# awentzonline/tartangan

Hardware: AMD Instinct MI355X
Metric: images/sec (G+D step) (higher is better)
Workload: dtype f32; 1 GPU; 128:3 SA-GAN cnn G+D step (R1 penalty, Adam x2, EMA), 128x128 RGB, batch 64/GPU, global batch 64; trainer=cnn, gan_config=128:3, global_batch=64, parallelism=dp1, hip_graphs=True

## Files before the change

tartangan_amd/csrc/conv.hip:

```cpp
#include <cstdlib>
#include <type_traits>
#include <utility>

#include "common.h"

namespace {

typedef float f32x16 __attribute__((ext_vector_type(16)));
typedef float f32x4 __attribute__((ext_vector_type(4)));

constexpr int CT_THREADS = 256;

template <int TH_, int TW_, int NI_>
struct Geo {
  static constexpr int TH = TH_, TW = TW_, NI = NI_, NPIX = TH_ * TW_ * NI_;
  static_assert(NPIX == 512 || NPIX == 256 || NPIX == 64, "a pixel tile is 512 / 256 pixels (waves split pixels) or 64 (waves split K)");
  static constexpr int PPW = (NPIX == 64) ? 64 : NPIX / 4;
  static_assert(TW_ % 4 == 0, "rows are staged as float4");
};
using G4 = Geo<4, 4, 16>;
using G8 = Geo<8, 8, 4>;
using G16 = Geo<16, 16, 1>;
using GX = Geo<8, 32, 1>;
using G4k = Geo<4, 4, 4>;
// ... 1033 lines not shown
  for (int n = 0; n < NT; ++n) {
    const int col = n * 16 + j;
    const int ci = col / KK, tap = col % KK;
    colbase[n] = (col < C::NCOL) ? (ci * P::CIS + (tap / KS) * P::PWS + (tap % KS)) : 0;
  }
  const int lane_b = pix_off<G, KS>(wave * 64) + h;
  const int lane_a = j * WG_GYS + wave * 64 + h;

  f32x4 acc[MTW][NT];
#pragma unroll
  for (int m = 0; m < MTW; ++m)
#pragma unroll
    for (int n = 0; n < NT; ++n) acc[m][n] = f32x4{0.f, 0.f, 0.f, 0.f};

  PatchStager<G, KS, CKW> ps;
  GyStager<G, CT> gs;
  const bool do_bias = (bias_part != nullptr) && (blockIdx.z == 0);
  float bsum[GyStager<G, CT>::NV];
#pragma unroll
  for (int i = 0; i < GyStager<G, CT>::NV; ++i) bsum[i] = 0.f;
  if (split < ntiles) {
    const TileCoord tc = decode_tile<G>(split, s.H, s.W);
    ps.load(x, s, s.Cin, ci0, tc, vec_x);
    gs.load(gy, s, co0, tc, vec_gy);
  }
  for (int t = split; t < ntiles; t += S) {
    __syncthreads();
    ps.store(pl);
    gs.store(gl);
    if (do_bias) gs.add_channel_sums(bsum);
    __syncthreads();
    if (t + S < ntiles) {
      const TileCoord tn = decode_tile<G>(t + S, s.H, s.W);
      ps.load(x, s, s.Cin, ci0, tn, vec_x);
      gs.load(gy, s, co0, tn, vec_gy);
    }
#pragma unroll
    for (int g = 0; g < 16; ++g) {
      constexpr int PPI = G::TH * G::TW;
      const int pg = 4 * g;
      const int goff = ((pg / PPI) * P::PH + (pg % PPI) / G::TW) * P::PWS + (pg % G::TW);
      float a[MTW], b[NT];
#pragma unroll
      for (int m = 0; m < MTW; ++m) a[m] = gl[lane_a + m * 16 * WG_GYS + 4 * g];
#pragma unroll
      for (int n = 0; n < NT; ++n) b[n] = pl[colbase[n] + lane_b + goff];
#pragma unroll
      for (int m = 0; m < MTW; ++m)
#pragma unroll
        for (int n = 0; n < NT; ++n) acc[m][n] = __builtin_amdgcn_mfma_f32_16x16x4f32(a[m], b[n], acc[m][n], 0, 0, 0);
    }
  }

  if (do_bias && lane == 0) {
#pragma unroll
    for (int i = 0; i < GyStager<G, CT>::NV; ++i) {
      const int co = co0 + 4 * i + wave;
      if (4 * i + wave < CT && co < s.Cout) bias_part[(int64_t)split * s.Cout + co] = bsum[i];
    }
  }
  __syncthreads();
  float* red = lds;
#pragma unroll
  for (int m = 0; m < MTW; ++m)
#pragma unroll
    for (int n = 0; n < NT; ++n)
#pragma unroll
      for (int r = 0; r < 4; ++r) red[(((wave * MTW + m) * NT + n) * 4 + r) * 64 + lane] = acc[m][n][r];
  __syncthreads();
  constexpr int PER_WAVE = MTW * NT * 4 * 64;
  for (int e = threadIdx.x; e < PER_WAVE; e += CT_THREADS) {
    const float v = (red[e] + red[PER_WAVE + e]) + (red[2 * PER_WAVE + e] + red[3 * PER_WAVE + e]);
    const int l = e & 63, q = e >> 6;
    const int r = q & 3, n = (q >> 2) % NT, m = (q >> 2) / NT;
    const int col = n * 16 + (l & 15);
    const int co = co0 + m * 16 + (l >> 4) * 4 + r;
    const int ci = ci0 + col / KK, tap = col % KK;
    if (col < C::NCOL && co < s.Cout && ci < s.Cin)
      part[(((int64_t)split * s.Cout + co) * s.Cin + ci) * KK + tap] = v;
  }
}

constexpr int WGD_GYQ = 65;
template <class G, int MTW, int CKW, bool DB>
__global__ void __launch_bounds__(CT_THREADS)
conv_wgrad_dma_kernel(const float* __restrict__ x, const float* __restrict__ gy, float* __restrict__ part,
                      float* __restrict__ bias_part , Shape s, int ntiles, int S) {
  static_assert(G::NPIX == 256 && WG_GYS == 4 * WGD_GYQ, "256-pixel tiles");
  using P = DPatch<G>;
  constexpr int KK = 9, CT = 16 * MTW, NCOL = CKW * KK, NT = (NCOL + 15) / 16;
  constexpr int PCH = CKW * P::CPC, GCH = CT * WGD_GYQ;
  constexpr int PCHP = dma_pad(PCH), GCHP = dma_pad(GCH);
  constexpr int NVP = (PCHP + CT_THREADS - 1) / CT_THREADS, NVG = (GCHP + CT_THREADS - 1) / CT_THREADS;
  constexpr int PBUF = PCHP * 4, BUF = PBUF + GCHP * 4;
  constexpr int RED = 4 * MTW * NT * 4 * 64 + 4 * CT;
  constexpr int LDSF = ((DB ? 2 : 1) * BUF > RED) ? (DB ? 2 : 1) * BUF : RED;
  __shared__ __attribute__((aligned(16))) float lds[LDSF];

  const int lane = threadIdx.x & 63, wave = wave_index();
  if (s.prio) __builtin_amdgcn_s_setprio(3);
  const int j = lane & 15, h = lane >> 4;
  const int co0 = blockIdx.y * CT, ci0 = blockIdx.z * CKW;
  const int split = blockIdx.x;
  const uint32_t HW = (uint32_t)(s.H * s.W);

  int colbase[NT];
#pragma unroll
  for (int n = 0; n < NT; ++n) {
    const int col = n * 16 + j;
    const int ci = col / KK, tap = col % KK;
    colbase[n] = (col < NCOL) ? (ci * P::CIS + (tap / 3) * P::PWS + (tap % 3)) : 0;
  }
  const int lane_b = P::pix(wave * 64) + h;
  const int lane_a = j * WG_GYS + wave * 64 + h;

  f32x4 acc[MTW][NT];
#pragma unroll
  for (int m = 0; m < MTW; ++m)
#pragma unroll
    for (int n = 0; n < NT; ++n) acc[m][n] = f32x4{0.f, 0.f, 0.f, 0.f};
  const bool do_bias = (bias_part != nullptr) && (blockIdx.z == 0);
  float bsum[MTW];
#pragma unroll
  for (int m = 0; m < MTW; ++m) bsum[m] = 0.f;

  const int cvalid = min(CKW, s.Cin - ci0);
  auto issue = [&](int t, float* buf) {
    const TileCoord tc = decode_tile<G>(t, s.H, s.W);
    const char* xb = reinterpret_cast<const char*>(x) + ((int64_t)tc.b0 * s.Cin + ci0) * HW * 4;
    const int64_t xbytes = ((int64_t)(s.B - tc.b0) * s.Cin - ci0) * HW * 4;
    const char* gb = reinterpret_cast<const char*>(gy) + ((int64_t)tc.b0 * s.Cout + co0) * HW * 4;
    const int64_t gbytes = ((int64_t)(s.B - tc.b0) * s.Cout - co0) * HW * 4;
    const __amdgpu_buffer_rsrc_t rx = __builtin_amdgcn_make_buffer_rsrc(const_cast<char*>(xb), 0, (int)xbytes, 0x00020000);
    const __amdgpu_buffer_rsrc_t rg = __builtin_amdgcn_make_buffer_rsrc(const_cast<char*>(gb), 0, (int)gbytes, 0x00020000);
#pragma unroll
    for (int i = 0; i < NVP; ++i) {
      const int e = i * CT_THREADS + threadIdx.x;
      const int ci = e / P::CPC, rem = e % P::CPC;
      const int row = rem / P::QR, q = rem % P::QR;
      const int img = row / P::PH, r = row % P::PH;
      const int hh = tc.h0 + r - 1, ww = tc.w0 - 4 + 4 * q;
      const bool ok = (rem < P::RAW / 4) && (ci < cvalid) && (tc.b0 + img < s.B) && (hh >= 0) && (hh < s.H) && (ww >= 0) && (ww < s.W);
      const uint32_t off = ok ? (__umul24(__umul24(img, s.Cin) + ci, HW) + __umul24(hh, s.W) + ww) << 2 : DMA_OOB;
      if ((i + 1) * CT_THREADS <= PCHP || i * CT_THREADS + wave * 64 < PCHP) dma16(rx, buf + (i * CT_THREADS + wave * 64) * 4, off);
    }
#pragma unroll
    for (int i = 0; i < NVG; ++i) {
      const int e = i * CT_THREADS + threadIdx.x;
      const int co = e / WGD_GYQ, q = e % WGD_GYQ;
      const int p = 4 * q;
      const int img = p / (G::TH * G::TW), rem = p % (G::TH * G::TW);
      const int hh = tc.h0 + rem / G::TW, ww = tc.w0 + rem % G::TW;
      const bool ok = (e < GCH) && (q < 64) && (co0 + co < s.Cout) && (tc.b0 + img < s.B) && (hh < s.H) && (ww < s.W);
      const uint32_t off = ok ? (__umul24(__umul24(img, s.Cout) + co, HW) + __umul24(hh, s.W) + ww) << 2 : DMA_OOB;
      if ((i + 1) * CT_THREADS <= GCHP || i * CT_THREADS + wave * 64 < GCHP) dma16(rg, buf + PBUF + (i * CT_THREADS + wave * 64) * 4, off);
    }
  };
  auto compute = [&](const float* buf) {
    const float* pl = buf;
    const float* gl = buf + PBUF;
    if (s.prio) __builtin_amdgcn_s_setprio(0);
#pragma unroll
    for (int g = 0; g < 16; ++g) {
      constexpr int PPI = G::TH * G::TW;
      const int pg = 4 * g;
      const int goff = ((pg / PPI) * P::PH + (pg % PPI) / G::TW) * P::PWS + (pg % G::TW);
      float a[MTW], b[NT];
#pragma unroll
      for (int m = 0; m < MTW; ++m) a[m] = gl[lane_a + m * 16 * WG_GYS + 4 * g];
#pragma unroll
      for (int n = 0; n < NT; ++n) b[n] = pl[colbase[n] + lane_b + goff];
#pragma unroll
      for (int m = 0; m < MTW; ++m) bsum[m] += a[m];
#pragma unroll
      for (int m = 0; m < MTW; ++m)
#pragma unroll
        for (int n = 0; n < NT; ++n) acc[m][n] = __builtin_amdgcn_mfma_f32_16x16x4f32(a[m], b[n], acc[m][n], 0, 0, 0);
    }
    if (s.prio) __builtin_amdgcn_s_setprio(3);
  };

  if constexpr (DB) {
    if (split < ntiles) issue(split, lds);
    int buf = 0;
    for (int t = split; t < ntiles; t += S) {
      asm volatile("s_waitcnt vmcnt(0)" ::: "memory");
      __syncthreads();
      if (t + S < ntiles) issue(t + S, lds + (buf ^ 1) * BUF);
      compute(lds + buf * BUF);
      buf ^= 1;
    }
  } else {
    for (int t = split; t < ntiles; t += S) {
      __syncthreads();
      issue(t, lds);
      asm volatile("s_waitcnt vmcnt(0)" ::: "memory");
      __syncthreads();
      compute(lds);
    }
  }

  __syncthreads();
  float* red = lds;
#pragma unroll
  for (int m = 0; m < MTW; ++m)
#pragma unroll
    for (int n = 0; n < NT; ++n)
#pragma unroll
      for (int r = 0; r < 4; ++r) red[(((wave * MTW + m) * NT + n) * 4 + r) * 64 + lane] = acc[m][n][r];
  constexpr int PER_WAVE = MTW * NT * 4 * 64;
  float* bred = lds + 4 * PER_WAVE;
  if (do_bias) {
#pragma unroll
    for (int m = 0; m < MTW; ++m) {
      float v = bsum[m];
      v += __shfl_xor(v, 16, 64);
      v += __shfl_xor(v, 32, 64);
      if (h == 0) bred[wave * CT + m * 16 + j] = v;
    }
  }
  __syncthreads();
  for (int e = threadIdx.x; e < PER_WAVE; e += CT_THREADS) {
    const float v = (red[e] + red[PER_WAVE + e]) + (red[2 * PER_WAVE + e] + red[3 * PER_WAVE + e]);
    const int l = e & 63, q = e >> 6;
    const int r = q & 3, n = (q >> 2) % NT, m = (q >> 2) / NT;
    const int col = n * 16 + (l & 15);
    const int co = co0 + m * 16 + (l >> 4) * 4 + r;
    const int ci = ci0 + col / KK, tap = col % KK;
    if (col < NCOL && co < s.Cout && ci < s.Cin)
      part[(((int64_t)split * s.Cout + co) * s.Cin + ci) * KK + tap] = v;
  }
  if (do_bias && threadIdx.x < CT && co0 + (int)threadIdx.x < s.Cout) {
    const int c = threadIdx.x;
    bias_part[(int64_t)split * s.Cout + co0 + c] = (bred[c] + bred[CT + c]) + (bred[2 * CT + c] + bred[3 * CT + c]);
  }
}

template <int MT, int NT>
__global__ void __launch_bounds__(256)
conv1x1_wgrad_stream_kernel(const float* __restrict__ x, ChanSegs gys, float* __restrict__ part,
                            float* __restrict__ bias_part , int Cin, int Cout, int HW, int64_t groups, int S) {
  __shared__ float red[4 * MT * NT * 4 * 64 + 4 * 16 * MT];
  const int lane = threadIdx.x & 63, wave = threadIdx.x >> 6, j = lane & 15, h = lane >> 4;
  const int co0 = blockIdx.y * 16 * MT, ci0 = blockIdx.z * 16 * NT, split = blockIdx.x;
  const int64_t g_begin = groups * split / S, g_end = groups * (split + 1) / S;
  const int64_t n = g_end - g_begin;
  const int64_t w_begin = g_begin + n * wave / 4, w_end = g_begin + n * (wave + 1) / 4;
  const int gpp = HW >> 4;
  int64_t arow[MT], brow[NT], aimg[MT];
  const float* abase[MT];
#pragma unroll
  for (int m = 0; m < MT; ++m) {
    const int co = min(co0 + 16 * m + j, Cout - 1), k = gys.find(co);
    abase[m] = gys.p[k];
// ... 894 lines not shown
                     float* __restrict__ bias_part , int bias_mode) {
  using P = Patch2x<G>;
  constexpr int CKW = S2_CKW, NT = S2_NT, CT = 16;
  constexpr int PATCH = CKW * P::CIS, GYT = CT * WG_GYS;
  constexpr int RED = 4 * NT * 4 * 64;
  constexpr int LDS_FLOATS = (PATCH + GYT) > RED ? (PATCH + GYT) : RED;
  __shared__ __attribute__((aligned(16))) float lds[LDS_FLOATS];
  float* pl = lds;
  float* gl = lds + PATCH;
  const int lane = threadIdx.x & 63, wave = threadIdx.x >> 6;
  const int j = lane & 15, h = lane >> 4;
  const int co0 = blockIdx.y * CT, ci0 = blockIdx.z * CKW;
  const int split = blockIdx.x;
  int colbase[NT];
#pragma unroll
  for (int n = 0; n < NT; ++n) colbase[n] = n * P::CIS + (j >> 2) * P::PWS + (j & 3);
  const int lane_b = P::pix(wave * 64) + 2 * h;
  const int lane_a = j * WG_GYS + wave * 64 + h;
  f32x4 acc[NT];
  float bsum_a = 0.f, bsum_b[NT];
#pragma unroll
  for (int n = 0; n < NT; ++n) { acc[n] = f32x4{0.f, 0.f, 0.f, 0.f}; bsum_b[n] = 0.f; }
  const bool do_bias = bias_part != nullptr && (bias_mode == 0 ? blockIdx.z == 0 : blockIdx.y == 0);
  auto products = [&](const float* pl, const float* gl, auto with_sums) {
#pragma unroll
    for (int g = 0; g < 16; ++g) {
      const int pg = 4 * g;
      const int goff = 2 * (pg / G::TW) * P::PWS + 2 * (pg % G::TW);
      const float a = gl[lane_a + 4 * g];
      float b[NT];
#pragma unroll
      for (int n = 0; n < NT; ++n) b[n] = pl[colbase[n] + lane_b + goff];
      if constexpr (decltype(with_sums)::value) {
        bsum_a += a;
#pragma unroll
        for (int n = 0; n < NT; ++n) bsum_b[n] += b[n];
      }
#pragma unroll
      for (int n = 0; n < NT; ++n) acc[n] = __builtin_amdgcn_mfma_f32_16x16x4f32(a, b[n], acc[n], 0, 0, 0);
    }
  };
  PatchStager2x<G, CKW> ps;
  GyStager<G, CT> gs;
  const int H2 = 2 * s.H, W2 = 2 * s.W;
  if (split < ntiles) {
    const TileCoord tc = decode_tile<G>(split, s.H, s.W);
    ps.load(hi, s.B, s.Cin, H2, W2, ci0, tc, vec_hi);
    gs.load(lo, s, co0, tc, vec_lo);
  }
  for (int t = split; t < ntiles; t += S) {
    __syncthreads();
    ps.store(pl);
    gs.store(gl);
    __syncthreads();
    if (t + S < ntiles) {
      const TileCoord tn = decode_tile<G>(t + S, s.H, s.W);
      ps.load(hi, s.B, s.Cin, H2, W2, ci0, tn, vec_hi);
      gs.load(lo, s, co0, tn, vec_lo);
    }
    if (do_bias) products(pl, gl, std::true_type{});
    else products(pl, gl, std::false_type{});
  }
  __syncthreads();
  float* red = lds;
#pragma unroll
  for (int n = 0; n < NT; ++n)
#pragma unroll
    for (int r = 0; r < 4; ++r) red[((wave * NT + n) * 4 + r) * 64 + lane] = acc[n][r];
  __syncthreads();
  constexpr int PER_WAVE = NT * 4 * 64;
  for (int e = threadIdx.x; e < PER_WAVE; e += CT_THREADS) {
    const float v = (red[e] + red[PER_WAVE + e]) + (red[2 * PER_WAVE + e] + red[3 * PER_WAVE + e]);
    const int l = e & 63, q = e >> 6;
    const int r = q & 3, n = q >> 2;
    const int co = co0 + (l >> 4) * 4 + r, ci = ci0 + n, tap = l & 15;
    if (co < s.Cout && ci < s.Cin) part[(((int64_t)split * s.Cout + co) * s.Cin + ci) * 16 + tap] = v;
  }
  if (do_bias) {
    __syncthreads();
    s2_bias_finish<NT>(red, bsum_a, bsum_b, bias_mode, bias_part, split, s.Cout, s.Cin, co0, ci0, lane, wave);
  }
}

template <class G>
__global__ void __launch_bounds__(CT_THREADS)
conv_wgrad_s2_dma_kernel(const float* __restrict__ hi, const float* __restrict__ lo, float* __restrict__ part, Shape s , int ntiles, int S, float* __restrict__ bias_part ,
                         int bias_mode) {
  static_assert(G::NPIX == 256, "256-pixel tiles");
  using P = DPatch2x<G>;
  constexpr int CKW = S2_CKW, NT = S2_NT, CT = 16;
  constexpr int PCH = CKW * P::CPC, GCH = CT * WGD_GYQ;
  constexpr int PCHP = dma_pad(PCH), GCHP = dma_pad(GCH);
  constexpr int NVP = (PCHP + CT_THREADS - 1) / CT_THREADS, NVG = (GCHP + CT_THREADS - 1) / CT_THREADS;
  constexpr int PBUF = PCHP * 4, BUF = PBUF + GCHP * 4;
  constexpr int RED = 4 * NT * 4 * 64;
  __shared__ __attribute__((aligned(16))) float lds[BUF > RED ? BUF : RED];
  const int lane = threadIdx.x & 63, wave = wave_index();
  if (s.prio) __builtin_amdgcn_s_setprio(3);
  const int j = lane & 15, h = lane >> 4;
  const int co0 = blockIdx.y * CT, ci0 = blockIdx.z * CKW;
  const int split = blockIdx.x;
  const int H2 = 2 * s.H, W2 = 2 * s.W;
  const uint32_t HW = (uint32_t)(s.H * s.W), HW2 = (uint32_t)(H2 * W2);
  int colbase[NT];
#pragma unroll
  for (int n = 0; n < NT; ++n) colbase[n] = n * P::CIS + (j >> 2) * P::PWS + (j & 3);
  const int lane_b = P::pix(wave * 64) + 2 * h;
  const int lane_a = j * WG_GYS + wave * 64 + h;
  f32x4 acc[NT];
  float bsum_a = 0.f, bsum_b[NT];
#pragma unroll
  for (int n = 0; n < NT; ++n) { acc[n] = f32x4{0.f, 0.f, 0.f, 0.f}; bsum_b[n] = 0.f; }
  const bool do_bias = bias_part != nullptr && (bias_mode == 0 ? blockIdx.z == 0 : blockIdx.y == 0);
  auto products = [&](const float* pl, const float* gl, auto with_sums) {
#pragma unroll
    for (int g = 0; g < 16; ++g) {
      const int pg = 4 * g;
      const int goff = 2 * (pg / G::TW) * P::PWS + 2 * (pg % G::TW);
      const float a = gl[lane_a + 4 * g];
      float b[NT];
#pragma unroll
      for (int n = 0; n < NT; ++n) b[n] = pl[colbase[n] + lane_b + goff];
      if constexpr (decltype(with_sums)::value) {
        bsum_a += a;
#pragma unroll
        for (int n = 0; n < NT; ++n) bsum_b[n] += b[n];
      }
#pragma unroll
      for (int n = 0; n < NT; ++n) acc[n] = __builtin_amdgcn_mfma_f32_16x16x4f32(a, b[n], acc[n], 0, 0, 0);
    }
  };
  const int cvalid = min(CKW, s.Cin - ci0);
  for (int t = split; t < ntiles; t += S) {
    const TileCoord tc = decode_tile<G>(t, s.H, s.W);
    const char* xb = reinterpret_cast<const char*>(hi) + ((int64_t)tc.b0 * s.Cin + ci0) * HW2 * 4;
    const int64_t xbytes = ((int64_t)(s.B - tc.b0) * s.Cin - ci0) * HW2 * 4;
    const char* gb = reinterpret_cast<const char*>(lo) + ((int64_t)tc.b0 * s.Cout + co0) * HW * 4;
    const int64_t gbytes = ((int64_t)(s.B - tc.b0) * s.Cout - co0) * HW * 4;
    const __amdgpu_buffer_rsrc_t rx = __builtin_amdgcn_make_buffer_rsrc(const_cast<char*>(xb), 0, (int)xbytes, 0x00020000);
    const __amdgpu_buffer_rsrc_t rg = __builtin_amdgcn_make_buffer_rsrc(const_cast<char*>(gb), 0, (int)gbytes, 0x00020000);
    __syncthreads();
#pragma unroll
    for (int i = 0; i < NVP; ++i) {
      const int e = i * CT_THREADS + threadIdx.x;
      const int ci = e / P::CPC, rem = e % P::CPC;
      const int row = rem / P::QR, q = rem % P::QR;
      const int img = row / P::PH, r = row % P::PH;
      const int hh = 2 * tc.h0 - 1 + r, ww = 2 * tc.w0 - 4 + 4 * q;
      const bool ok = (rem < P::RAW / 4) && (ci < cvalid) && (tc.b0 + img < s.B) && (hh >= 0) && (hh < H2) && (ww >= 0) && (ww < W2);
      const uint32_t off = ok ? (__umul24(__umul24(img, s.Cin) + ci, HW2) + __umul24(hh, W2) + ww) << 2 : DMA_OOB;
      if ((i + 1) * CT_THREADS <= PCHP || i * CT_THREADS + wave * 64 < PCHP) dma16(rx, lds + (i * CT_THREADS + wave * 64) * 4, off);
    }
#pragma unroll
    for (int i = 0; i < NVG; ++i) {
      const int e = i * CT_THREADS + threadIdx.x;
      const int co = e / WGD_GYQ, q = e % WGD_GYQ;
      const int p = 4 * q;
      const int img = p / (G::TH * G::TW), rem = p % (G::TH * G::TW);
      const int hh = tc.h0 + rem / G::TW, ww = tc.w0 + rem % G::TW;
      const bool ok = (e < GCH) && (q < 64) && (co0 + co < s.Cout) && (tc.b0 + img < s.B) && (hh < s.H) && (ww < s.W);
      const uint32_t off = ok ? (__umul24(__umul24(img, s.Cout) + co, HW) + __umul24(hh, s.W) + ww) << 2 : DMA_OOB;
      if ((i + 1) * CT_THREADS <= GCHP || i * CT_THREADS + wave * 64 < GCHP) dma16(rg, lds + PBUF + (i * CT_THREADS + wave * 64) * 4, off);
    }
    asm volatile("s_waitcnt vmcnt(0)" ::: "memory");
    __syncthreads();
    const float* pl = lds;
    const float* gl = lds + PBUF;
    if (s.prio) __builtin_amdgcn_s_setprio(0);
    if (do_bias) products(pl, gl, std::true_type{});
    else products(pl, gl, std::false_type{});
    if (s.prio) __builtin_amdgcn_s_setprio(3);
  }
  __syncthreads();
  float* red = lds;
#pragma unroll
  for (int n = 0; n < NT; ++n)
#pragma unroll
    for (int r = 0; r < 4; ++r) red[((wave * NT + n) * 4 + r) * 64 + lane] = acc[n][r];
  __syncthreads();
  constexpr int PER_WAVE = NT * 4 * 64;
  for (int e = threadIdx.x; e < PER_WAVE; e += CT_THREADS) {
    const float v = (red[e] + red[PER_WAVE + e]) + (red[2 * PER_WAVE + e] + red[3 * PER_WAVE + e]);
    const int l = e & 63, q = e >> 6;
    const int r = q & 3, n = q >> 2;
    const int co = co0 + (l >> 4) * 4 + r, ci = ci0 + n, tap = l & 15;
    if (co < s.Cout && ci < s.Cin) part[(((int64_t)split * s.Cout + co) * s.Cin + ci) * 16 + tap] = v;
  }
  if (do_bias) {
    __syncthreads();
    s2_bias_finish<NT>(red, bsum_a, bsum_b, bias_mode, bias_part, split, s.Cout, s.Cin, co0, ci0, lane, wave);
  }
}

__device__ __forceinline__ void s2wgrad_reduce_fold(const float* __restrict__ part, float* __restrict__ gw, int S, int Clo, int Chi,
                                                    int Cout, int Cin, int mode, int accumulate,
                                                    const float* __restrict__ bias_part , float* __restrict__ gbias,
                                                    int pair_blocks, int bx ) {
  if (bx >= pair_blocks) {
    const int c = (bx - pair_blocks) * 4 + (threadIdx.x >> 6), lane = threadIdx.x & 63;
    if (c >= Cout) return;
    float v = 0.f;
    for (int sidx = lane; sidx < S; sidx += 64) v += bias_part[(int64_t)sidx * Cout + c];
#pragma unroll
    for (int m = 32; m >= 1; m >>= 1) v += __shfl_xor(v, m, 64);
    if (lane == 0) gbias[c] = accumulate ? gbias[c] + v : v;
    return;
  }
  __shared__ float red[4][4][16];
  __shared__ float T[4][16];
  const int tap = threadIdx.x & 15, pr = (threadIdx.x >> 4) & 3, sl = threadIdx.x >> 6;
  const int64_t npairs = (int64_t)Clo * Chi;
  const int64_t pair = (int64_t)bx * 4 + pr;
  float a0 = 0.f, a1 = 0.f;
  if (pair < npairs) {
    const float* src = part + pair * 16 + tap;
    const int64_t stride = npairs * 16;
    int s = sl;
    for (; s + 4 < S; s += 8) { a0 += src[(int64_t)s * stride]; a1 += src[(int64_t)(s + 4) * stride]; }
    for (; s < S; s += 4) a0 += src[(int64_t)s * stride];
  }
  red[sl][pr][tap] = a0 + a1;
  __syncthreads();
  if (sl == 0) T[pr][tap] = (red[0][pr][tap] + red[1][pr][tap]) + (red[2][pr][tap] + red[3][pr][tap]);
  __syncthreads();
  if (threadIdx.x < 36) {
    const int p = threadIdx.x / 9, k = threadIdx.x % 9, kh = k / 3, kw = k % 3;
    const int64_t pp = (int64_t)bx * 4 + p;
    if (pp < npairs) {
      const int lo = (int)(pp / Chi), hi = (int)(pp % Chi);
      const int co = mode == 0 ? lo : hi, ci = mode == 0 ? hi : lo;
      const int u0 = mode == 0 ? kh : 2 - kh, v0 = mode == 0 ? kw : 2 - kw;
      float r = (T[p][u0 * 4 + v0] + T[p][u0 * 4 + v0 + 1]) + (T[p][(u0 + 1) * 4 + v0] + T[p][(u0 + 1) * 4 + v0 + 1]);
      if (mode == 0) r *= 0.25f;
      float* o = gw + ((int64_t)co * Cin + ci) * 9 + k;
      *o = accumulate ? *o + r : r;
    }
  }
}

__global__ void __launch_bounds__(256) s2wgrad_reduce_fold_kernel(const float* __restrict__ part, float* __restrict__ gw, int S, int Clo,
                                                                  int Chi, int Cout, int Cin, int mode, int accumulate,
                                                                  const float* __restrict__ bias_part, float* __restrict__ gbias,
                                                                  int pair_blocks) {
  s2wgrad_reduce_fold(part, gw, S, Clo, Chi, Cout, Cin, mode, accumulate, bias_part, gbias, pair_blocks, (int)blockIdx.x);
}
constexpr int SB_MAX_ITEMS = 16;
// ... 367 lines not shown
                              int64_t min_wgs) {
  if (s.Cin % 16 != 0) return -1;
  const int tiles = num_tiles<G>(s.B, s.H, s.W);
  const int flags = (tiles % 8 == 0) ? 1 : 0;
  if (s.Cout > 16 && (int64_t)tiles * ((s.Cout + 31) / 32) >= 256 && s.B % 2 == 0)
    conv_wino_dma_kernel<G, 2, DGRAD, 16, true><<<dim3(tiles, (s.Cout + 31) / 32), CT_THREADS, 0, st>>>(x, w, bias, residual, y, s, flags);
  else if ((int64_t)tiles * ((s.Cout + 15) / 16) >= min_wgs)
    conv_wino_dma_kernel<G, 1, DGRAD, 16, true><<<dim3(tiles, (s.Cout + 15) / 16), CT_THREADS, 0, st>>>(x, w, bias, residual, y, s, flags);
  else
    return -1;
  return tg_launch_status();
}
template <bool DGRAD>
static bool try_launch_wino(const float* x, const float* w, const float* bias, const float* residual, float* y, Shape s, hipStream_t st,
                            int* rc) {
  const int mode = wino_mode();
  if (!mode) return false;
  if (s.os != 1 || (s.Cin % WINO_CK != 0 && s.Cin != 4) || s.Cout < 4 || s.W % 4 != 0 || !tg_aligned16(x) || !tg_aligned16(y) ||
      (residual && !tg_aligned16(residual)) || (int64_t)s.B * s.Cin * s.H * s.W * 4 >= (1ll << 31))
    return false;
  const int64_t min_wgs = (mode == 2) ? 1 : 256;
  int r = -1;
  if (s.H % 8 == 0 && s.W % 32 == 0) r = launch_wino_geo<GX, DGRAD>(x, w, bias, residual, y, s, st, min_wgs);
  else if (s.H == 16 && s.W == 16) r = launch_wino_geo<G16, DGRAD>(x, w, bias, residual, y, s, st, mode == 2 ? 1 : 512);
  else if (mode == 2 && s.H == 8 && s.W == 8) r = launch_wino_ksplit<G8k, DGRAD>(x, w, bias, residual, y, s, st, min_wgs);
  else if (mode == 2 && s.H == 4 && s.W == 4) r = launch_wino_ksplit<G4k, DGRAD>(x, w, bias, residual, y, s, st, min_wgs);
  if (r < 0) return false;
  *rc = r;
  return true;
}

template <int KS, bool DGRAD>
int launch_fwd(const float* x, const float* w, const float* bias, const float* residual, float* y, Shape s, hipStream_t st) {
  if constexpr (KS == 3) {
    int rc = 0;
    if (try_launch_wino<DGRAD>(x, w, bias, residual, y, s, st, &rc)) return rc;
    if (try_launch_dma<DGRAD>(x, w, bias, residual, y, s, st, &rc)) return rc;
  }
  if constexpr (KS == 1) {
    const int mode = conv1x1_mode();
    if (mode != 0 && conv1x1_mfma_ok(x, residual, y, s) && (mode == 2 || (!conv1x1_direct_ok(s) && s.Cin <= 32)))
      return launch_conv1x1_mfma(x, w, bias, residual, y, s, DGRAD, st);
    if (conv1x1_direct_ok(s)) return launch_conv1x1(x, w, bias, residual, y, s, DGRAD, st);
  }
  const GeoId g = pick_geo(s.H, s.W);
  const int64_t wgs256 = (int64_t)geo_tiles(g, s.B, s.H, s.W) * ((s.Cout + 63) / 64);
  const bool ksplit = (g != GEO_X) && wgs256 < 128 && s.Cin >= 16;
  switch (g) {
    case GEO_4: return ksplit ? launch_fwd_geo<G4k, KS, DGRAD>(x, w, bias, residual, y, s, st) : launch_fwd_geo<G4, KS, DGRAD>(x, w, bias, residual, y, s, st);
    case GEO_8: return ksplit ? launch_fwd_geo<G8k, KS, DGRAD>(x, w, bias, residual, y, s, st) : launch_fwd_geo<G8, KS, DGRAD>(x, w, bias, residual, y, s, st);
    case GEO_16: return ksplit ? launch_fwd_geo<G16k, KS, DGRAD>(x, w, bias, residual, y, s, st) : launch_fwd_geo<G16, KS, DGRAD>(x, w, bias, residual, y, s, st);
    default: return launch_fwd_geo<GX, KS, DGRAD>(x, w, bias, residual, y, s, st);
  }
}

struct WgPlan {
  int tiles, co_tiles, ci_chunks, S, mtw;
};
static inline WgPlan wgrad_plan(int B, int Cin, int Cout, int H, int W, int ks) {
  WgPlan p;
  p.tiles = geo_tiles(pick_geo(H, W), B, H, W);
  p.mtw = (Cout > 16 && H * W == 64) ? 2 : 1;
  p.co_tiles = (Cout + 16 * p.mtw - 1) / (16 * p.mtw);
  const int ckw = (ks == 3) ? WgCfg<3>::CKW : WgCfg<1>::CKW;
  p.ci_chunks = (Cin + ckw - 1) / ckw;
  const int groups = p.co_tiles * p.ci_chunks;
  int S = 768 / groups;
  const int smax = p.tiles >= 4096 ? 512 : 256;
  if (S > smax) S = smax;
  if (S < 1) S = 1;
  if (S > p.tiles) S = p.tiles;
  p.S = S;
  return p;
}

template <class G, int KS>
int launch_wgrad_geo(const float* x, const float* gy, float* part, float* bias_part, Shape s, const WgPlan& p, hipStream_t st) {
  dim3 grid(p.S, p.co_tiles, p.ci_chunks);
  const int vx = plane_vec_ok(x, s.W), vg = plane_vec_ok(gy, s.W);
  if constexpr (KS == 3 && G::NPIX == 256) {
    const DmaKnobs& k = dma_knobs();
    const bool small = (int64_t)s.B * (s.Cin > s.Cout ? s.Cin : s.Cout) * s.H * s.W * 4 < (1ll << 31);
    constexpr int CKW = WgCfg<3>::CKW;
    constexpr int buf1 = (dma_pad(CKW * DPatch<G>::CPC) + dma_pad(16 * WGD_GYQ)) * 16, buf2 = (dma_pad(CKW * DPatch<G>::CPC) + dma_pad(32 * WGD_GYQ)) * 16;
    if (k.enable && k.wgrad && vx && vg && small) {
      s.prio = k.prio;
      const bool db = k.wgrad_db == 1 || (k.wgrad_db < 0 && p.tiles >= 2 * p.S && (int64_t)p.S * p.co_tiles * p.ci_chunks <= 600);
      if (s.Cin <= 4 && p.mtw == 1) {
        conv_wgrad_dma_kernel<G, 1, 4, false><<<grid, CT_THREADS, 0, st>>>(x, gy, part, bias_part, s, p.tiles, p.S);
        return tg_launch_status();
      }
      if (p.mtw == 2) {
        if constexpr (2 * buf2 <= 160 * 1024) {
          if (db) { conv_wgrad_dma_kernel<G, 2, CKW, true><<<grid, CT_THREADS, 0, st>>>(x, gy, part, bias_part, s, p.tiles, p.S); return tg_launch_status(); }
        }
        if constexpr (buf2 <= 160 * 1024) {
          conv_wgrad_dma_kernel<G, 2, CKW, false><<<grid, CT_THREADS, 0, st>>>(x, gy, part, bias_part, s, p.tiles, p.S);
          return tg_launch_status();
        }
      } else {
        if constexpr (2 * buf1 <= 160 * 1024) {
          if (db) { conv_wgrad_dma_kernel<G, 1, CKW, true><<<grid, CT_THREADS, 0, st>>>(x, gy, part, bias_part, s, p.tiles, p.S); return tg_launch_status(); }
        }
        if constexpr (buf1 <= 160 * 1024) {
          conv_wgrad_dma_kernel<G, 1, CKW, false><<<grid, CT_THREADS, 0, st>>>(x, gy, part, bias_part, s, p.tiles, p.S);
          return tg_launch_status();
        }
      }
    }
  }
  if constexpr (KS == 1) {
    if (conv1x1_wgrad_stream_ok(x, gy, s)) return launch_conv1x1_wgrad_stream(x, gy, part, bias_part, s, p.S, st);
  }
  if (p.mtw == 2) conv_wgrad_kernel<G, KS, 2><<<grid, CT_THREADS, 0, st>>>(x, gy, part, bias_part, s, p.tiles, p.S, vx, vg);
  else conv_wgrad_kernel<G, KS, 1><<<grid, CT_THREADS, 0, st>>>(x, gy, part, bias_part, s, p.tiles, p.S, vx, vg);
  return tg_launch_status();
}

template <int KS>
int launch_wgrad(const float* x, const float* gy, float* part, float* bias_part, Shape s, const WgPlan& p, hipStream_t st) {
  switch (pick_geo(s.H, s.W)) {
    case GEO_4: return launch_wgrad_geo<G4, KS>(x, gy, part, bias_part, s, p, st);
    case GEO_8: return launch_wgrad_geo<G8, KS>(x, gy, part, bias_part, s, p, st);
    case GEO_16: return launch_wgrad_geo<G16, KS>(x, gy, part, bias_part, s, p, st);
    default: return launch_wgrad_geo<GX, KS>(x, gy, part, bias_part, s, p, st);
  }
}

static inline int check_shape(int B, int Cin, int Cout, int H, int W, int ks) {
  if (B <= 0 || Cin <= 0 || Cout <= 0 || H <= 0 || W <= 0) return TG_EINVAL;
  if (ks != 1 && ks != 3) return TG_EUNSUPPORTED;
  if ((int64_t)B * (Cin > Cout ? Cin : Cout) * H * W >= (1ll << 40)) return TG_EUNSUPPORTED;
  const int64_t ni = (H == 4 && W == 4) ? 16 : (H == 8 && W == 8) ? 4 : 1;
  const int64_t cmax = Cin > Cout ? Cin : Cout;
  if ((int64_t)H * W >= (1 << 24) || cmax * 9 >= (1 << 24) || ni * cmax * H * W >= (1ll << 30)) return TG_EUNSUPPORTED;
  return TG_OK;
}

}

extern "C" {

int tg_conv2d_fwd(const float* x, const float* w, const float* bias, const float* residual, float* y, int B, int Cin, int Cout,
                  int H, int W, int ks, void* stream) {
  TG_CHECK_PTR(x); TG_CHECK_PTR(w); TG_CHECK_PTR(y);
  if (int rc = check_shape(B, Cin, Cout, H, W, ks)) return rc;
  Shape s{B, Cin, Cout, H, W};
  return ks == 3 ? launch_fwd<3, false>(x, w, bias, residual, y, s, tg_stream(stream))
                 : launch_fwd<1, false>(x, w, bias, residual, y, s, tg_stream(stream));
}

int tg_conv2d_fwd_up2res(const float* x, const float* w, const float* bias, const float* residual_lo, float* y, int B, int Cin,
                         int Cout, int H, int W, void* stream) {
  TG_CHECK_PTR(x); TG_CHECK_PTR(w); TG_CHECK_PTR(y); TG_CHECK_PTR(residual_lo);
  if (int rc = check_shape(B, Cin, Cout, H, W, 3)) return rc;
  if ((H & 1) || (W & 1)) return TG_EUNSUPPORTED;
  Shape s{B, Cin, Cout, H, W};
  s.res_up = 1;
  return launch_fwd<3, false>(x, w, bias, residual_lo, y, s, tg_stream(stream));
}

int tg_upconv3x3_weights(const float* w, float* wp, int Cout, int Cin, void* stream) {
  TG_CHECK_PTR(w); TG_CHECK_PTR(wp); TG_CHECK_POS(Cout); TG_CHECK_POS(Cin);
  const int n = Cout * Cin;
  upconv_weights_kernel<<<(n + 255) / 256, 256, 0, tg_stream(stream)>>>(w, wp, n);
  return tg_launch_status();
}
// ... 368 lines not shown
```

Baseline: 6986 images/s.

## Rebuild wgrad LDS patch layout to remove bank conflicts and hoist DMA addressing

```diff
diff --git a/tartangan_amd/csrc/conv.hip b/tartangan_amd/csrc/conv.hip
--- a/tartangan_amd/csrc/conv.hip
+++ b/tartangan_amd/csrc/conv.hip
@@ -1139,12 +1139,82 @@
 }
 
 constexpr int WGD_GYQ = 65;
+
+struct WgConflicts { int worst, excess; };
+constexpr WgConflicts wg_b_conflicts(int PWS, int SK, int CIS, int CKW) {
+  const int NCOL = CKW * 9, NT = (NCOL + 15) / 16, PAIR = 2 * PWS + SK;
+  WgConflicts res{1, 0};
+  for (int par = 0; par < (SK ? 2 : 1); ++par)
+    for (int n = 0; n < NT; ++n) {
+      int addr[32] = {}, on_bank[32] = {};
+      for (int i = 0; i < 32; ++i) {
+        const int col = n * 16 + i / 2, ky = (col % 9) / 3;
+        const int rowoff = ky == 0 ? 0 : ky == 1 ? PWS + par * SK : PAIR;
+        addr[i] = (col < NCOL ? (col / 9) * CIS + rowoff + (col % 9) % 3 : 0) + i % 2;
+        bool first = true;
+        for (int k = 0; k < i && first; ++k) first = addr[k] != addr[i];
+        if (first) ++on_bank[addr[i] % 32];
+      }
+      int deg = 1;
+      for (int bank = 0; bank < 32; ++bank)
+        if (on_bank[bank] > deg) deg = on_bank[bank];
+      res.excess += deg - 1;
+      if (deg > res.worst) res.worst = deg;
+    }
+  return res;
+}
+constexpr int wg_pick_cis(int PWS, int SK, int RAW) {
+  int best = RAW, best_excess = 1 << 30;
+  for (int cis = RAW; cis < RAW + 32; cis += 4) {
+    const int e = wg_b_conflicts(PWS, SK, cis, 16).excess + wg_b_conflicts(PWS, SK, cis, 4).excess;
+    if (e < best_excess) { best = cis; best_excess = e; }
+  }
+  return best;
+}
+template <class G> struct WgPatch {
+  static constexpr int PH = G::TH + 2, PWS = G::TW + 8, QR = PWS / 4;
+  static constexpr int SK = (2 * PWS) % 32 == 0 ? 4 : 0;
+  static constexpr int PAIR = 2 * PWS + SK, PAIRQ = PAIR / 4;
+  static constexpr int IMG = (PH / 2) * PAIR, RAW = G::NI * IMG;
+  static constexpr int CIS = wg_pick_cis(PWS, SK, RAW);
+  static constexpr int CPC = CIS / 4;
+  static_assert(PH % 2 == 0 && CIS % 4 == 0 && CIS >= RAW, "row pairs, whole chunks");
+  static_assert(SK == 0 || 64 % (G::TH * G::TW) == 0 || (64 / G::TW) % 2 == 0, "row parity per k-group");
+  __host__ __device__ static constexpr int row_off(int R) { return (R / 2) * PAIR + (R % 2) * PWS; }
+  __host__ __device__ static constexpr int tap_off(int ky, int par) { return row_off(par + ky) - row_off(par); }
+  __device__ __forceinline__ static int pix(int p) {
+    const int img = p / (G::TH * G::TW), rem = p % (G::TH * G::TW);
+    return img * IMG + row_off(rem / G::TW) + rem % G::TW + 3;
+  }
+  static constexpr WgConflicts C16 = wg_b_conflicts(PWS, SK, CIS, 16), C4 = wg_b_conflicts(PWS, SK, CIS, 4);
+};
+static_assert(WgPatch<GX>::CIS == 412 && WgPatch<GX>::C16.worst == 1 && WgPatch<GX>::C4.worst == 1, "GX: conflict-free B reads");
+static_assert(WgPatch<G16>::CIS == 436 && WgPatch<G16>::C16.worst == 1 && WgPatch<G16>::C4.worst == 1, "G16: conflict-free B reads");
+static_assert(WgPatch<G4>::CIS == 1156 && WgPatch<G4>::C16.worst == 1 && WgPatch<G4>::C4.worst == 1, "G4: conflict-free B reads");
+static_assert(WgPatch<G8>::CIS == 728 && WgPatch<G8>::C16.worst == 2 && WgPatch<G8>::C16.excess == 6 && WgPatch<G8>::C4.excess == 1,
+              "G8: 2-way on the three-channel N-tiles only (6 of the 18 (row parity, N-tile) pairs)");
+static_assert(wg_b_conflicts(DPatch<GX>::PWS, 0, DPatch<GX>::CIS, 16).excess == 9 && wg_b_conflicts(DPatch<G8>::PWS, 0, DPatch<G8>::CIS, 16).worst == 3,
+              "what DPatch's strides gave these reads: every N-tile 2-way (GX), 3-way (G8)");
+
+struct DmaChunk { uint32_t rel, key; };
+struct DmaWindow { uint32_t ka, kb, origin; };
+__device__ __forceinline__ DmaChunk dma_chunk(bool ok, uint32_t rel, int q, int r, int img) {
+  return DmaChunk{rel, ok ? (uint32_t)(q | (r << 8) | (img << 16)) : (127u << 16)};
+}
+__device__ __forceinline__ DmaWindow dma_window(int qlo, int qhi, int rlo, int rhi, int nimg, uint32_t origin) {
+  return DmaWindow{(uint32_t)((0x80 - qlo) | ((0x80 - rlo) << 8) | (0x80 << 16)), (uint32_t)((0x7f + qhi) | ((0x7f + rhi) << 8) | ((0x7f + nimg) << 16)), origin};
+}
+__device__ __forceinline__ uint32_t dma_off(const DmaChunk& c, const DmaWindow& w) {
+  const uint32_t in = (c.key + w.ka) & (w.kb - c.key) & 0x808080u;
+  return in == 0x808080u ? c.rel + w.origin : DMA_OOB;
+}
+
 template <class G, int MTW, int CKW, bool DB>
 __global__ void __launch_bounds__(CT_THREADS)
 conv_wgrad_dma_kernel(const float* __restrict__ x, const float* __restrict__ gy, float* __restrict__ part,
                       float* __restrict__ bias_part , Shape s, int ntiles, int S) {
   static_assert(G::NPIX == 256 && WG_GYS == 4 * WGD_GYQ, "256-pixel tiles");
-  using P = DPatch<G>;
+  using P = WgPatch<G>;
   constexpr int KK = 9, CT = 16 * MTW, NCOL = CKW * KK, NT = (NCOL + 15) / 16;
   constexpr int PCH = CKW * P::CPC, GCH = CT * WGD_GYQ;
   constexpr int PCHP = dma_pad(PCH), GCHP = dma_pad(GCH);
@@ -1161,12 +1231,13 @@
   const int split = blockIdx.x;
   const uint32_t HW = (uint32_t)(s.H * s.W);
 
-  int colbase[NT];
+  int colbase[NT], colbase_odd[NT];
 #pragma unroll
   for (int n = 0; n < NT; ++n) {
     const int col = n * 16 + j;
     const int ci = col / KK, tap = col % KK;
-    colbase[n] = (col < NCOL) ? (ci * P::CIS + (tap / 3) * P::PWS + (tap % 3)) : 0;
+    colbase[n] = (col < NCOL) ? (ci * P::CIS + P::tap_off(tap / 3, 0) + (tap % 3)) : 0;
+    colbase_odd[n] = (col < NCOL) ? (ci * P::CIS + P::tap_off(tap / 3, 1) + (tap % 3)) : 0;
   }
   const int lane_b = P::pix(wave * 64) + h;
   const int lane_a = j * WG_GYS + wave * 64 + h;
@@ -1182,36 +1253,42 @@
   for (int m = 0; m < MTW; ++m) bsum[m] = 0.f;
 
   const int cvalid = min(CKW, s.Cin - ci0);
+  const __amdgpu_buffer_rsrc_t rx = __builtin_amdgcn_make_buffer_rsrc(
+      const_cast<char*>(reinterpret_cast<const char*>(x)) + (int64_t)ci0 * HW * 4, 0, (int)(((int64_t)s.B * s.Cin - ci0) * HW * 4), 0x00020000);
+  const __amdgpu_buffer_rsrc_t rg = __builtin_amdgcn_make_buffer_rsrc(
+      const_cast<char*>(reinterpret_cast<const char*>(gy)) + (int64_t)co0 * HW * 4, 0, (int)(((int64_t)s.B * s.Cout - co0) * HW * 4), 0x00020000);
+  DmaChunk pc[NVP], gc[NVG];
+#pragma unroll
+  for (int i = 0; i < NVP; ++i) {
+    const int e = i * CT_THREADS + threadIdx.x;
+    const int ci = e / P::CPC, rem = e % P::CPC;
+    const int img = rem / (P::IMG / 4), u = rem % (P::IMG / 4) % P::PAIRQ;
+    const int r = 2 * (rem % (P::IMG / 4) / P::PAIRQ) + (u >= P::QR ? 1 : 0), q = (u >= P::QR) ? u - P::QR : u;
+    const bool ok = (rem < P::RAW / 4) && (q < P::QR) && (ci < cvalid);
+    pc[i] = dma_chunk(ok, (uint32_t)((int)(__umul24(__umul24(img, s.Cin) + ci, HW) + __umul24(r, s.W)) - s.W + 4 * q - 4) << 2, q, r, img);
+  }
+#pragma unroll
+  for (int i = 0; i < NVG; ++i) {
+    const int e = i * CT_THREADS + threadIdx.x;
+    const int co = e / WGD_GYQ, q = e % WGD_GYQ;
+    const int p = 4 * q;
+    const int img = p / (G::TH * G::TW), rem = p % (G::TH * G::TW);
+    const bool ok = (e < GCH) && (q < 64) && (co0 + co < s.Cout);
+    gc[i] = dma_chunk(ok, (__umul24(__umul24(img, s.Cout) + co, HW) + __umul24(rem / G::TW, s.W) + rem % G::TW) << 2, (rem % G::TW) / 4, rem / G::TW, img);
+  }
   auto issue = [&](int t, float* buf) {
     const TileCoord tc = decode_tile<G>(t, s.H, s.W);
-    const char* xb = reinterpret_cast<const char*>(x) + ((int64_t)tc.b0 * s.Cin + ci0) * HW * 4;
-    const int64_t xbytes = ((int64_t)(s.B - tc.b0) * s.Cin - ci0) * HW * 4;
-    const char* gb = reinterpret_cast<const char*>(gy) + ((int64_t)tc.b0 * s.Cout + co0) * HW * 4;
-    const int64_t gbytes = ((int64_t)(s.B - tc.b0) * s.Cout - co0) * HW * 4;
-    const __amdgpu_buffer_rsrc_t rx = __builtin_amdgcn_make_buffer_rsrc(const_cast<char*>(xb), 0, (int)xbytes, 0x00020000);
-    const __amdgpu_buffer_rsrc_t rg = __builtin_amdgcn_make_buffer_rsrc(const_cast<char*>(gb), 0, (int)gbytes, 0x00020000);
-#pragma unroll
-    for (int i = 0; i < NVP; ++i) {
-      const int e = i * CT_THREADS + threadIdx.x;
-      const int ci = e / P::CPC, rem = e % P::CPC;
-      const int row = rem / P::QR, q = rem % P::QR;
-      const int img = row / P::PH, r = row % P::PH;
-      const int hh = tc.h0 + r - 1, ww = tc.w0 - 4 + 4 * q;
-      const bool ok = (rem < P::RAW / 4) && (ci < cvalid) && (tc.b0 + img < s.B) && (hh >= 0) && (hh < s.H) && (ww >= 0) && (ww < s.W);
-      const uint32_t off = ok ? (__umul24(__umul24(img, s.Cin) + ci, HW) + __umul24(hh, s.W) + ww) << 2 : DMA_OOB;
-      if ((i + 1) * CT_THREADS <= PCHP || i * CT_THREADS + wave * 64 < PCHP) dma16(rx, buf + (i * CT_THREADS + wave * 64) * 4, off);
-    }
-#pragma unroll
-    for (int i = 0; i < NVG; ++i) {
-      const int e = i * CT_THREADS + threadIdx.x;
-      const int co = e / WGD_GYQ, q = e % WGD_GYQ;
-      const int p = 4 * q;
-      const int img = p / (G::TH * G::TW), rem = p % (G::TH * G::TW);
-      const int hh = tc.h0 + rem / G::TW, ww = tc.w0 + rem % G::TW;
-      const bool ok = (e < GCH) && (q < 64) && (co0 + co < s.Cout) && (tc.b0 + img < s.B) && (hh < s.H) && (ww < s.W);
-      const uint32_t off = ok ? (__umul24(__umul24(img, s.Cout) + co, HW) + __umul24(hh, s.W) + ww) << 2 : DMA_OOB;
-      if ((i + 1) * CT_THREADS <= GCHP || i * CT_THREADS + wave * 64 < GCHP) dma16(rg, buf + PBUF + (i * CT_THREADS + wave * 64) * 4, off);
-    }
+    const int colq = (s.W - tc.w0) >> 2, nimg = min(G::NI, s.B - tc.b0);
+    const uint32_t org = (uint32_t)(tc.h0 * s.W + tc.w0) << 2;
+    const DmaWindow wx = dma_window(tc.w0 == 0 ? 1 : 0, min(P::QR, colq + 1), tc.h0 == 0 ? 1 : 0, min(P::PH, s.H + 1 - tc.h0), nimg,
+                                    (((uint32_t)(tc.b0 * s.Cin) * HW) << 2) + org);
+    const DmaWindow wg = dma_window(0, min(G::TW / 4, colq), 0, min(G::TH, s.H - tc.h0), nimg, (((uint32_t)(tc.b0 * s.Cout) * HW) << 2) + org);
+#pragma unroll
+    for (int i = 0; i < NVP; ++i)
+      if ((i + 1) * CT_THREADS <= PCHP || i * CT_THREADS + wave * 64 < PCHP) dma16(rx, buf + (i * CT_THREADS + wave * 64) * 4, dma_off(pc[i], wx));
+#pragma unroll
+    for (int i = 0; i < NVG; ++i)
+      if ((i + 1) * CT_THREADS <= GCHP || i * CT_THREADS + wave * 64 < GCHP) dma16(rg, buf + PBUF + (i * CT_THREADS + wave * 64) * 4, dma_off(gc[i], wg));
   };
   auto compute = [&](const float* buf) {
     const float* pl = buf;
@@ -1221,12 +1298,13 @@
     for (int g = 0; g < 16; ++g) {
       constexpr int PPI = G::TH * G::TW;
       const int pg = 4 * g;
-      const int goff = ((pg / PPI) * P::PH + (pg % PPI) / G::TW) * P::PWS + (pg % G::TW);
+      const int prow = (pg % PPI) / G::TW;
+      const int goff = (pg / PPI) * P::IMG + P::row_off(prow) + (pg % G::TW);
       float a[MTW], b[NT];
 #pragma unroll
       for (int m = 0; m < MTW; ++m) a[m] = gl[lane_a + m * 16 * WG_GYS + 4 * g];
 #pragma unroll
-      for (int n = 0; n < NT; ++n) b[n] = pl[colbase[n] + lane_b + goff];
+      for (int n = 0; n < NT; ++n) b[n] = pl[((P::SK != 0 && (prow & 1)) ? colbase_odd[n] : colbase[n]) + lane_b + goff];
 #pragma unroll
       for (int m = 0; m < MTW; ++m) bsum[m] += a[m];
 #pragma unroll
@@ -2287,6 +2365,23 @@
   }
 }
 
+constexpr int s2_b_conflicts(int PWS) {
+  int deg = 1;
+  for (int grp = 0; grp < 4; grp += 2)
+    for (int bank = 0; bank < 32; ++bank) {
+      int distinct = 0;
+      for (int i = 0; i < 32; ++i) {
+        const int ai = (i / 2 >> 2) * PWS + (i / 2 & 3) + 2 * (grp + i % 2);
+        bool first = ai % 32 == bank;
+        for (int k = 0; k < i; ++k) first = first && ((k / 2 >> 2) * PWS + (k / 2 & 3) + 2 * (grp + k % 2)) != ai;
+        distinct += first;
+      }
+      if (distinct > deg) deg = distinct;
+    }
+  return deg;
+}
+static_assert(s2_b_conflicts(DPatch2x<GX>::PWS) == 1 && s2_b_conflicts(DPatch2x<G16>::PWS) == 1 && s2_b_conflicts(DPatch2x<G8>::PWS) == 1,
+              "conv_wgrad_s2_dma_kernel: conflict-free B reads");
 template <class G>
 __global__ void __launch_bounds__(CT_THREADS)
 conv_wgrad_s2_dma_kernel(const float* __restrict__ hi, const float* __restrict__ lo, float* __restrict__ part, Shape s , int ntiles, int S, float* __restrict__ bias_part ,
@@ -2336,37 +2431,43 @@
     }
   };
   const int cvalid = min(CKW, s.Cin - ci0);
+  const __amdgpu_buffer_rsrc_t rx = __builtin_amdgcn_make_buffer_rsrc(
+      const_cast<char*>(reinterpret_cast<const char*>(hi)) + (int64_t)ci0 * HW2 * 4, 0, (int)(((int64_t)s.B * s.Cin - ci0) * HW2 * 4), 0x00020000);
+  const __amdgpu_buffer_rsrc_t rg = __builtin_amdgcn_make_buffer_rsrc(
+      const_cast<char*>(reinterpret_cast<const char*>(lo)) + (int64_t)co0 * HW * 4, 0, (int)(((int64_t)s.B * s.Cout - co0) * HW * 4), 0x00020000);
+  DmaChunk pc[NVP], gc[NVG];
+#pragma unroll
+  for (int i = 0; i < NVP; ++i) {
+    const int e = i * CT_THREADS + threadIdx.x;
+    const int ci = e / P::CPC, rem = e % P::CPC;
+    const int row = rem / P::QR, q = rem % P::QR;
+    const int img = row / P::PH, r = row % P::PH;
+    const bool ok = (rem < P::RAW / 4) && (ci < cvalid);
+    pc[i] = dma_chunk(ok, (uint32_t)((int)(__umul24(__umul24(img, s.Cin) + ci, HW2) + __umul24(r, W2)) - W2 + 4 * q - 4) << 2, q, r, img);
+  }
+#pragma unroll
+  for (int i = 0; i < NVG; ++i) {
+    const int e = i * CT_THREADS + threadIdx.x;
+    const int co = e / WGD_GYQ, q = e % WGD_GYQ;
+    const int p = 4 * q;
+    const int img = p / (G::TH * G::TW), rem = p % (G::TH * G::TW);
+    const bool ok = (e < GCH) && (q < 64) && (co0 + co < s.Cout);
+    gc[i] = dma_chunk(ok, (__umul24(__umul24(img, s.Cout) + co, HW) + __umul24(rem / G::TW, s.W) + rem % G::TW) << 2, (rem % G::TW) / 4, rem / G::TW, img);
+  }
   for (int t = split; t < ntiles; t += S) {
     const TileCoord tc = decode_tile<G>(t, s.H, s.W);
-    const char* xb = reinterpret_cast<const char*>(hi) + ((int64_t)tc.b0 * s.Cin + ci0) * HW2 * 4;
-    const int64_t xbytes = ((int64_t)(s.B - tc.b0) * s.Cin - ci0) * HW2 * 4;
-    const char* gb = reinterpret_cast<const char*>(lo) + ((int64_t)tc.b0 * s.Cout + co0) * HW * 4;
-    const int64_t gbytes = ((int64_t)(s.B - tc.b0) * s.Cout - co0) * HW * 4;
-    const __amdgpu_buffer_rsrc_t rx = __builtin_amdgcn_make_buffer_rsrc(const_cast<char*>(xb), 0, (int)xbytes, 0x00020000);
-    const __amdgpu_buffer_rsrc_t rg = __builtin_amdgcn_make_buffer_rsrc(const_cast<char*>(gb), 0, (int)gbytes, 0x00020000);
+    const int colq = (s.W - tc.w0) >> 2, nimg = min(G::NI, s.B - tc.b0);
+    const DmaWindow wx = dma_window(tc.w0 == 0 ? 1 : 0, min(P::QR, 2 * colq + 1), tc.h0 == 0 ? 1 : 0, min(P::PH, H2 + 1 - 2 * tc.h0), nimg,
+                                    (((uint32_t)(tc.b0 * s.Cin) * HW2) << 2) + ((uint32_t)(2 * tc.h0 * W2 + 2 * tc.w0) << 2));
+    const DmaWindow wg = dma_window(0, min(G::TW / 4, colq), 0, min(G::TH, s.H - tc.h0), nimg,
+                                    (((uint32_t)(tc.b0 * s.Cout) * HW) << 2) + ((uint32_t)(tc.h0 * s.W + tc.w0) << 2));
     __syncthreads();
 #pragma unroll
-    for (int i = 0; i < NVP; ++i) {
-      const int e = i * CT_THREADS + threadIdx.x;
-      const int ci = e / P::CPC, rem = e % P::CPC;
-      const int row = rem / P::QR, q = rem % P::QR;
-      const int img = row / P::PH, r = row % P::PH;
-      const int hh = 2 * tc.h0 - 1 + r, ww = 2 * tc.w0 - 4 + 4 * q;
-      const bool ok = (rem < P::RAW / 4) && (ci < cvalid) && (tc.b0 + img < s.B) && (hh >= 0) && (hh < H2) && (ww >= 0) && (ww < W2);
-      const uint32_t off = ok ? (__umul24(__umul24(img, s.Cin) + ci, HW2) + __umul24(hh, W2) + ww) << 2 : DMA_OOB;
-      if ((i + 1) * CT_THREADS <= PCHP || i * CT_THREADS + wave * 64 < PCHP) dma16(rx, lds + (i * CT_THREADS + wave * 64) * 4, off);
-    }
-#pragma unroll
-    for (int i = 0; i < NVG; ++i) {
-      const int e = i * CT_THREADS + threadIdx.x;
-      const int co = e / WGD_GYQ, q = e % WGD_GYQ;
-      const int p = 4 * q;
-      const int img = p / (G::TH * G::TW), rem = p % (G::TH * G::TW);
-      const int hh = tc.h0 + rem / G::TW, ww = tc.w0 + rem % G::TW;
-      const bool ok = (e < GCH) && (q < 64) && (co0 + co < s.Cout) && (tc.b0 + img < s.B) && (hh < s.H) && (ww < s.W);
-      const uint32_t off = ok ? (__umul24(__umul24(img, s.Cout) + co, HW) + __umul24(hh, s.W) + ww) << 2 : DMA_OOB;
-      if ((i + 1) * CT_THREADS <= GCHP || i * CT_THREADS + wave * 64 < GCHP) dma16(rg, lds + PBUF + (i * CT_THREADS + wave * 64) * 4, off);
-    }
+    for (int i = 0; i < NVP; ++i)
+      if ((i + 1) * CT_THREADS <= PCHP || i * CT_THREADS + wave * 64 < PCHP) dma16(rx, lds + (i * CT_THREADS + wave * 64) * 4, dma_off(pc[i], wx));
+#pragma unroll
+    for (int i = 0; i < NVG; ++i)
+      if ((i + 1) * CT_THREADS <= GCHP || i * CT_THREADS + wave * 64 < GCHP) dma16(rg, lds + PBUF + (i * CT_THREADS + wave * 64) * 4, dma_off(gc[i], wg));
     asm volatile("s_waitcnt vmcnt(0)" ::: "memory");
     __syncthreads();
     const float* pl = lds;
@@ -2900,7 +3001,9 @@
     const DmaKnobs& k = dma_knobs();
     const bool small = (int64_t)s.B * (s.Cin > s.Cout ? s.Cin : s.Cout) * s.H * s.W * 4 < (1ll << 31);
     constexpr int CKW = WgCfg<3>::CKW;
-    constexpr int buf1 = (dma_pad(CKW * DPatch<G>::CPC) + dma_pad(16 * WGD_GYQ)) * 16, buf2 = (dma_pad(CKW * DPatch<G>::CPC) + dma_pad(32 * WGD_GYQ)) * 16;
+    constexpr int buf1 = (dma_pad(CKW * WgPatch<G>::CPC) + dma_pad(16 * WGD_GYQ)) * 16, buf2 = (dma_pad(CKW * WgPatch<G>::CPC) + dma_pad(32 * WGD_GYQ)) * 16;
+    constexpr int old1 = (dma_pad(CKW * DPatch<G>::CPC) + dma_pad(16 * WGD_GYQ)) * 16, old2 = (dma_pad(CKW * DPatch<G>::CPC) + dma_pad(32 * WGD_GYQ)) * 16;
+    static_assert(160 * 1024 / buf1 >= 160 * 1024 / old1 && 160 * 1024 / buf2 >= 160 * 1024 / old2, "workgroups per CU by LDS");
     if (k.enable && k.wgrad && vx && vg && small) {
       s.prio = k.prio;
       const bool db = k.wgrad_db == 1 || (k.wgrad_db < 0 && p.tiles >= 2 * p.S && (int64_t)p.S * p.co_tiles * p.ci_chunks <= 600);
```

New measurement: 7069 images/s (median of 6 runs). 1.01x the previous value.
